# msg7086/x265-Yuuki-Asuna

Measured on AMD Instinct MI355X. Metric: encoded fps + bit-exact check, 4K preset=slow, 1/2/4/8 MI355X vs host AVX2, higher is better.
Workload: dtype u8; 1 GPU; 3840x2160 8-bit closed-loop frame pipeline (tier T2): lookahead -> exhaustive +-57 ME, 85 PUs/CTU -> subme 3 -> MC + DCT/quant/recon qp 27 -> deblock -> SAO (rdo) -> border -> next reference; parallelism=none (1 GPU), ctus_per_frame=2040

## Files before the change

x265-yuuki-asuna_amd/csrc/phase_kernels.hip:

```cpp
#include "common.h"
#include "tile_interp.h"

#include <cstdlib>

namespace x265hip {

struct PhaseArgs
{
    const uint8_t* src;
    uint8_t* dst;
    long strideB;
    int rows, tilesW, depth;
    size_t planeBytes;
};

__constant__ int8_t kPhaseChromaTaps[8][4] = {
    { 0, 64, 0, 0 }, { -2, 58, 10, -2 }, { -4, 54, 16, -2 }, { -6, 46, 28, -4 },
    { -4, 36, 36, -4 }, { -4, 28, 46, -6 }, { -2, 16, 54, -4 }, { -2, 10, 58, -2 } };

template <typename Px> __device__ __forceinline__ void phase_store(uint8_t* out, long strideB, const int (&d)[4][4])
{
#pragma unroll
    for (int y = 0; y < 4; y++)
    {
        uint32_t* o = reinterpret_cast<uint32_t*>(out + y * strideB);
        if (sizeof(Px) == 1)
            o[0] = (uint32_t)d[y][0] | ((uint32_t)d[y][1] << 8) | ((uint32_t)d[y][2] << 16) | ((uint32_t)d[y][3] << 24);
        else
        {
            o[0] = (uint32_t)d[y][0] | ((uint32_t)d[y][1] << 16);
            o[1] = (uint32_t)d[y][2] | ((uint32_t)d[y][3] << 16);
        }
    }
}

template <typename Px>
__global__ void __launch_bounds__(256) phase_luma_kernel(PhaseArgs a)
{
    constexpr int BPP = sizeof(Px);
    int bx, by;
    xcd_swizzle_2d(bx, by);
    const int tx = bx * 256 + threadIdx.x, ty = by + 1;
    if (tx >= a.tilesW) return;
    const long off = (long)(ty * 4) * a.strideB + (long)tx * 4 * BPP;
    const uint8_t* org = a.src + off;
    const int maxVal = (1 << a.depth) - 1, headRoom = 14 - a.depth;
    const int shiftPS = 6 - headRoom, offPS = -(8192 << shiftPS);
    const int shiftSP = 6 + headRoom, offSP = (1 << (shiftSP - 1)) + (8192 << 6);
    auto vtaps = [](const int yf, uint32_t (&cv)[4])
    {
        cv[0] = tile_sel3(yf, 0x0004ffffu, 0x0004ffffu, 0x00010000u); cv[1] = tile_sel3(yf, 0x003afff6u, 0x0028fff5u, 0x0011fffbu);
        cv[2] = tile_sel3(yf, 0xfffb0011u, 0xfff50028u, 0xfff6003au); cv[3] = tile_sel3(yf, 0x00000001u, 0xffff0004u, 0xffff0004u);
    };
#pragma unroll
    for (int xf = 0; xf < 4; xf++)
    {
        int col[11][4];
#pragma unroll
        for (int t = 0; t < 11; t++)
        {
            const uint8_t* rp = org + (long)(t - 3) * a.strideB;
            if (xf == 0)
            {
                if (BPP == 1) { const uint32_t w = ld_u32(rp); col[t][0] = w & 0xff; col[t][1] = (w >> 8) & 0xff; col[t][2] = (w >> 16) & 0xff; col[t][3] = w >> 24; }
                else { const uint32_t w0 = ld_u32(rp), w1 = ld_u32(rp + 4); col[t][0] = w0 & 0xffff; col[t][1] = w0 >> 16; col[t][2] = w1 & 0xffff; col[t][3] = w1 >> 16; }
            }
            else
                tile_hrow<BPP>(rp - 3 * BPP, xf, col[t]);
        }
        int d[4][4];
        if (xf)
        {
#pragma unroll
            for (int y = 0; y < 4; y++)
#pragma unroll
                for (int x = 0; x < 4; x++) d[y][x] = tile_clip16((col[y + 3][x] + 32) >> 6, maxVal);
            phase_store<Px>(a.dst + (size_t)(xf - 1) * a.planeBytes + off, a.strideB, d);
        }
        uint32_t pairs[10][4];
#pragma unroll
        for (int t = 0; t < 10; t++)
#pragma unroll
            for (int x = 0; x < 4; x++)
            {
                const uint32_t lo = xf ? (uint32_t)((col[t][x] + offPS) >> shiftPS) : (uint32_t)col[t][x];
                const uint32_t hi = xf ? (uint32_t)((col[t + 1][x] + offPS) >> shiftPS) : (uint32_t)col[t + 1][x];
                pairs[t][x] = __builtin_amdgcn_perm(hi, lo, 0x05040100u);
            }
#pragma unroll
        for (int yf = 1; yf < 4; yf++)
        {
            uint32_t cv[4];
            vtaps(yf, cv);
#pragma unroll
            for (int y = 0; y < 4; y++)
#pragma unroll
                for (int x = 0; x < 4; x++)
                {
                    int sum = 0;
#pragma unroll
                    for (int j = 0; j < 4; j++) sum = tile_dot2(pairs[y + 2 * j][x], cv[j], sum);
                    d[y][x] = xf ? tile_clip16((sum + offSP) >> shiftSP, maxVal) : tile_clip16((sum + 32) >> 6, maxVal);
                }
            phase_store<Px>(a.dst + (size_t)(yf * 4 + xf - 1) * a.planeBytes + off, a.strideB, d);
        }
    }
}

__device__ __forceinline__ uint32_t quad_xor1(uint32_t v) { return (uint32_t)dpp<0xB1>((int)v); }
__device__ __forceinline__ uint32_t quad_xor2(uint32_t v) { return (uint32_t)dpp<0x4E>((int)v); }

__device__ __forceinline__ void quad_transpose4(uint32_t (&p)[4], int l)
{
    const bool o1 = l & 1, o2 = l & 2;
    {
        const uint32_t a = quad_xor1(o1 ? p[0] : p[1]), b = quad_xor1(o1 ? p[2] : p[3]);
        if (o1) { p[0] = a; p[2] = b; } else { p[1] = a; p[3] = b; }
    }
    {
        const uint32_t a = quad_xor2(o2 ? p[0] : p[2]), b = quad_xor2(o2 ? p[1] : p[3]);
        if (o2) { p[0] = a; p[1] = b; } else { p[2] = a; p[3] = b; }
    }
}

template <typename Px> __device__ __forceinline__ void phase_store_wide(uint8_t* plane, long strideB, int ty, int tx, int lane, const int (&d)[4][4])
{
    if (sizeof(Px) == 1)
    {
        uint32_t p[4];
#pragma unroll
        for (int y = 0; y < 4; y++) p[y] = (uint32_t)d[y][0] | ((uint32_t)d[y][1] << 8) | ((uint32_t)d[y][2] << 16) | ((uint32_t)d[y][3] << 24);
        quad_transpose4(p, lane);
        uint4* o = reinterpret_cast<uint4*>(plane + (long)(ty * 4 + (lane & 3)) * strideB + (long)(tx & ~3) * 4);
        *o = make_uint4(p[0], p[1], p[2], p[3]);
    }
    else
    {
        uint32_t lo[4], hi[4];
#pragma unroll
        for (int y = 0; y < 4; y++) { lo[y] = (uint32_t)d[y][0] | ((uint32_t)d[y][1] << 16); hi[y] = (uint32_t)d[y][2] | ((uint32_t)d[y][3] << 16); }
        const bool odd = lane & 1;
#pragma unroll
        for (int r = 0; r < 4; r += 2)
        {
            const uint32_t sl = quad_xor1(odd ? lo[r] : lo[r + 1]), sh = quad_xor1(odd ? hi[r] : hi[r + 1]);
            const uint4 v = odd ? make_uint4(sl, sh, lo[r + 1], hi[r + 1]) : make_uint4(lo[r], hi[r], sl, sh);
            uint4* o = reinterpret_cast<uint4*>(plane + (long)(ty * 4 + r + (odd ? 1 : 0)) * strideB + (long)(tx & ~1) * 8);
            *o = v;
        }
    }
}

template <int BPP> __device__ __forceinline__ void tile_hrow_regs(const uint32_t* w, int xf, int (&out)[4])
{
    if (BPP == 1)
    {
        const uint32_t c03 = tile_sel3(xf, 0x3af604ffu, 0x28f504ffu, 0x11fb0100u), c47 = tile_sel3(xf, 0x0001fb11u, 0xff04f528u, 0xff04f63au);
        const uint32_t w0 = w[0] ^ 0x80808080u, w1 = w[1] ^ 0x80808080u, w2 = w[2] ^ 0x80808080u;
#pragma unroll
        for (int x = 0; x < 4; x++)
        {
            const uint32_t lo = x ? __builtin_amdgcn_alignbyte(w1, w0, x) : w0, hi = x ? __builtin_amdgcn_alignbyte(w2, w1, x) : w1;
            out[x] = __builtin_amdgcn_sdot4((int)hi, (int)c47, __builtin_amdgcn_sdot4((int)lo, (int)c03, 8192, false), false);
        }
    }
    else
    {
        const uint32_t cp[4] = { tile_sel3(xf, 0x0004ffffu, 0x0004ffffu, 0x00010000u), tile_sel3(xf, 0x003afff6u, 0x0028fff5u, 0x0011fffbu),
                                 tile_sel3(xf, 0xfffb0011u, 0xfff50028u, 0xfff6003au), tile_sel3(xf, 0x00000001u, 0xffff0004u, 0xffff0004u) };
#pragma unroll
        for (int x = 0; x < 4; x++)
        {
            int sacc = 0;
#pragma unroll
            for (int j = 0; j < 4; j++)
            {
                const int k = (x >> 1) + j;
                sacc = tile_dot2((x & 1) ? __builtin_amdgcn_alignbyte(w[k + 1], w[k], 2) : w[k], cp[j], sacc);
            }
            out[x] = sacc;
        }
    }
}

template <typename Px, bool XF0>
__device__ __forceinline__ void phase_column_set(const PhaseArgs& a, const uint32_t (&raw)[11][sizeof(Px) == 1 ? 3 : 6], int xf, int ty, int tx, int lane, bool live)
{
    constexpr int BPP = sizeof(Px);
    const int maxVal = (1 << a.depth) - 1, headRoom = 14 - a.depth;
    const int shiftPS = 6 - headRoom, offPS = -(8192 << shiftPS);
    const int shiftSP = 6 + headRoom, offSP = (1 << (shiftSP - 1)) + (8192 << 6);
    int d[4][4];
    uint32_t pairs[10][4], prev[4] = { 0, 0, 0, 0 };
#pragma unroll
    for (int t = 0; t < 11; t++)
    {
        int col[4];
        if (XF0)
        {
            if (BPP == 1)
            {
                const uint32_t w = __builtin_amdgcn_alignbyte(raw[t][1], raw[t][0], 3);
                col[0] = w & 0xff; col[1] = (w >> 8) & 0xff; col[2] = (w >> 16) & 0xff; col[3] = w >> 24;
            }
            else
            {
                col[0] = raw[t][1] >> 16; col[1] = raw[t][2] & 0xffff; col[2] = raw[t][2] >> 16; col[3] = raw[t][3] & 0xffff;
            }
        }
        else
        {
            tile_hrow_regs<BPP>(raw[t], xf, col);
            if (t >= 3 && t < 7)
#pragma unroll
                for (int x = 0; x < 4; x++) d[t - 3][x] = tile_clip16((col[x] + 32) >> 6, maxVal);
        }
#pragma unroll
        for (int x = 0; x < 4; x++)
        {
            const uint32_t cur = XF0 ? (uint32_t)col[x] : (uint32_t)((col[x] + offPS) >> shiftPS);
            if (t) pairs[t - 1][x] = __builtin_amdgcn_perm(cur, prev[x], 0x05040100u);
            prev[x] = cur;
        }
    }
    if (!XF0 && live) phase_store_wide<Px>(a.dst + (size_t)(xf - 1) * a.planeBytes, a.strideB, ty, tx, lane, d);
#pragma unroll 1
    for (int yf = 1; yf < 4; yf++)
    {
        const uint32_t cv[4] = { tile_sel3(yf, 0x0004ffffu, 0x0004ffffu, 0x00010000u), tile_sel3(yf, 0x003afff6u, 0x0028fff5u, 0x0011fffbu),
                                 tile_sel3(yf, 0xfffb0011u, 0xfff50028u, 0xfff6003au), tile_sel3(yf, 0x00000001u, 0xffff0004u, 0xffff0004u) };
#pragma unroll
        for (int y = 0; y < 4; y++)
#pragma unroll
            for (int x = 0; x < 4; x++)
            {
                int sum = 0;
#pragma unroll
                for (int j = 0; j < 4; j++) sum = tile_dot2(pairs[y + 2 * j][x], cv[j], sum);
                d[y][x] = XF0 ? tile_clip16((sum + 32) >> 6, maxVal) : tile_clip16((sum + offSP) >> shiftSP, maxVal);
            }
        if (live) phase_store_wide<Px>(a.dst + (size_t)(yf * 4 + xf - 1) * a.planeBytes, a.strideB, ty, tx, lane, d);
    }
}

template <typename Px>
__device__ __forceinline__ void phase_luma_wide_body(const PhaseArgs& a)
{
    constexpr int BPP = sizeof(Px), NW = BPP == 1 ? 3 : 6;
    const int lane = threadIdx.x & 63;
    int bx, by;
    xcd_swizzle_2d(bx, by);
    const int tx = bx * 256 + threadIdx.x, ty = by + 1;
    const bool live = tx < a.tilesW;
    const int txl = live ? tx : a.tilesW - 4 + (tx & 3);
    const uint8_t* org = a.src + (long)(ty * 4) * a.strideB + (long)txl * 4 * BPP;
    uint32_t raw[11][NW];
#pragma unroll
    for (int t = 0; t < 11; t++)
#pragma unroll
        for (int k = 0; k < NW; k++) raw[t][k] = ld_u32(org + (long)(t - 3) * a.strideB - 3 * BPP + 4 * k);
    phase_column_set<Px, true>(a, raw, 0, ty, tx, lane, live);
#pragma unroll 1
    for (int xf = 1; xf < 4; xf++)
        phase_column_set<Px, false>(a, raw, xf, ty, tx, lane, live);
}
template <typename Px> __global__ void __launch_bounds__(256) phase_luma_wide_kernel(PhaseArgs a) { phase_luma_wide_body<Px>(a); }

template <typename Px>
__global__ void __launch_bounds__(256) phase_chroma_kernel(PhaseArgs a)
{
    constexpr int BPP = sizeof(Px);
    int bx, by;
    xcd_swizzle_2d(bx, by);
    const int tx = bx * 256 + threadIdx.x, ty = by + 1;
    if (tx >= a.tilesW) return;
    const long off = (long)(ty * 4) * a.strideB + (long)tx * 4 * BPP;
    const int maxVal = (1 << a.depth) - 1, headRoom = 14 - a.depth;
    const int shiftPS = 6 - headRoom, offPS = -(8192 << shiftPS);
    const int shiftSP = 6 + headRoom, offSP = (1 << (shiftSP - 1)) + (8192 << 6);
    int s[7][7];
#pragma unroll
    for (int r = 0; r < 7; r++)
    {
        const uint8_t* rp = a.src + off + (long)(r - 1) * a.strideB - BPP;
        if (BPP == 1)
        {
            const uint32_t w0 = ld_u32(rp), w1 = ld_u32(rp + 4);
            s[r][0] = w0 & 0xff; s[r][1] = (w0 >> 8) & 0xff; s[r][2] = (w0 >> 16) & 0xff; s[r][3] = w0 >> 24;
            s[r][4] = w1 & 0xff; s[r][5] = (w1 >> 8) & 0xff; s[r][6] = (w1 >> 16) & 0xff;
        }
        else
        {
            const uint32_t w0 = ld_u32(rp), w1 = ld_u32(rp + 4), w2 = ld_u32(rp + 8), w3 = ld_u32(rp + 12);
            s[r][0] = w0 & 0xffff; s[r][1] = w0 >> 16; s[r][2] = w1 & 0xffff; s[r][3] = w1 >> 16;
            s[r][4] = w2 & 0xffff; s[r][5] = w2 >> 16; s[r][6] = w3 & 0xffff;
        }
    }
#pragma unroll 1
    for (int xf = 0; xf < 8; xf++)
    {
        const int cx0 = kPhaseChromaTaps[xf][0], cx1 = kPhaseChromaTaps[xf][1], cx2 = kPhaseChromaTaps[xf][2], cx3 = kPhaseChromaTaps[xf][3];
        int col[7][4];
#pragma unroll
        for (int r = 0; r < 7; r++)
#pragma unroll
            for (int x = 0; x < 4; x++)
                col[r][x] = xf ? cx0 * s[r][x] + cx1 * s[r][x + 1] + cx2 * s[r][x + 2] + cx3 * s[r][x + 3] : s[r][x + 1];
        int d[4][4];
        if (xf)
        {
#pragma unroll
            for (int y = 0; y < 4; y++)
#pragma unroll
                for (int x = 0; x < 4; x++) d[y][x] = tile_clip16((col[y + 1][x] + 32) >> 6, maxVal);
            phase_store<Px>(a.dst + (size_t)(xf - 1) * a.planeBytes + off, a.strideB, d);
#pragma unroll
            for (int r = 0; r < 7; r++)
#pragma unroll
                for (int x = 0; x < 4; x++) col[r][x] = (int16_t)((col[r][x] + offPS) >> shiftPS);
        }
#pragma unroll 1
        for (int yf = 1; yf < 8; yf++)
        {
            const int cy0 = kPhaseChromaTaps[yf][0], cy1 = kPhaseChromaTaps[yf][1], cy2 = kPhaseChromaTaps[yf][2], cy3 = kPhaseChromaTaps[yf][3];
#pragma unroll
            for (int y = 0; y < 4; y++)
#pragma unroll
                for (int x = 0; x < 4; x++)
                {
                    const int sum = cy0 * col[y][x] + cy1 * col[y + 1][x] + cy2 * col[y + 2][x] + cy3 * col[y + 3][x];
                    d[y][x] = xf ? tile_clip16((sum + offSP) >> shiftSP, maxVal) : tile_clip16((sum + 32) >> 6, maxVal);
                }
            phase_store<Px>(a.dst + (size_t)(yf * 8 + xf - 1) * a.planeBytes + off, a.strideB, d);
        }
    }
}

}

using namespace x265hip;

int x265hip::phase_planes_launch(int depth, int chroma, const void* src, void* dst, intptr_t stride, int rows, size_t plane_bytes, hipStream_t s)
{
    const int bpp = depth == 8 ? 1 : 2;
    PhaseArgs a;
    a.src = (const uint8_t*)src; a.dst = (uint8_t*)dst; a.strideB = (long)stride * bpp; a.rows = rows;
    a.tilesW = (int)(stride / 4); a.depth = depth; a.planeBytes = plane_bytes;
    const dim3 gridL((a.tilesW + 255) / 256, rows / 4 - 3);
    if (chroma)
    {
        if (bpp == 1) hipLaunchKernelGGL(phase_chroma_kernel<uint8_t>, gridL, dim3(256), 0, s, a);
        else hipLaunchKernelGGL(phase_chroma_kernel<uint16_t>, gridL, dim3(256), 0, s, a);
    }
    else
    {
        static const int force = getenv("X265HIP_PHASE_KERNEL") ? atoi(getenv("X265HIP_PHASE_KERNEL")) : 0;
        const bool wideOk = !(a.tilesW & 3) && !(((uintptr_t)dst | plane_bytes) & 15);
        const bool wide = wideOk && (force == 2 || (force != 1 && bpp == 2));
        if (wide)
        {
            if (bpp == 1) hipLaunchKernelGGL(phase_luma_wide_kernel<uint8_t>, gridL, dim3(256), 0, s, a);
            else hipLaunchKernelGGL(phase_luma_wide_kernel<uint16_t>, gridL, dim3(256), 0, s, a);
        }
        else if (bpp == 1) hipLaunchKernelGGL(phase_luma_kernel<uint8_t>, gridL, dim3(256), 0, s, a);
        else hipLaunchKernelGGL(phase_luma_kernel<uint16_t>, gridL, dim3(256), 0, s, a);
    }
    return check_hip(hipGetLastError(), "phase_planes launch");
}

extern "C" int x265hip_phase_planes(const x265hip_phase_planes_params* p, void* stream)
{
    if (!p || !p->src || !p->dst) { set_error("phase_planes: NULL argument"); return X265HIP_EINVAL; }
    if (p->depth != 8 && p->depth != 10 && p->depth != 12) { set_error("phase_planes: depth %d", p->depth); return X265HIP_EINVAL; }
    const int bpp = p->depth == 8 ? 1 : 2;
    if (p->stride <= 0 || p->rows <= 0 || (p->rows & 3) || ((p->stride * bpp) & 3) || (p->stride & 3))
    { set_error("phase_planes: stride %ld / rows %d must be positive multiples of 4", (long)p->stride, p->rows); return X265HIP_EINVAL; }
    if ((uintptr_t)p->dst & 3) { set_error("phase_planes: dst must be 4-byte aligned"); return X265HIP_EINVAL; }
    if (p->rows / 4 > 65535 || p->rows < 16) { set_error("phase_planes: %d rows", p->rows); return X265HIP_EINVAL; }
    int rc = ensure_device();
    if (rc) return rc;
    return phase_planes_launch(p->depth, p->chroma, p->src, p->dst, p->stride, p->rows, (size_t)p->stride * p->rows * bpp, (hipStream_t)stream);
}
```

Measured before the change: 659.4 frames/s.

## Add dedicated 8-bit luma phase kernel using packed dot products

Adds a specialized 8-bit luma subpel phase-plane kernel that computes horizontal filters with sdot4 on byte-aligned words and vertical filters with sdot2 on packed 16-bit pairs. It uses packed arithmetic-shift-clip-to-u8 instructions to produce all 15 phase planes in one pass over an 11-row window. This is meant to replace the generic templated per-pixel arithmetic for the default 8-bit path and cut ALU and register cost. The risk is bit-exactness in the bias and offset handling, plus higher register pressure from the pairs array.

Measured after the change: 673.0 frames/s (median of 6 runs). 2.1% higher.

```diff
diff --git a/x265-yuuki-asuna_amd/csrc/phase_kernels.hip b/x265-yuuki-asuna_amd/csrc/phase_kernels.hip
--- a/x265-yuuki-asuna_amd/csrc/phase_kernels.hip
+++ b/x265-yuuki-asuna_amd/csrc/phase_kernels.hip
@@ -266,6 +266,85 @@
 }
 template <typename Px> __global__ void __launch_bounds__(256) phase_luma_wide_kernel(PhaseArgs a) { phase_luma_wide_body<Px>(a); }
 
+typedef unsigned short phase_v2u16 __attribute__((ext_vector_type(2)));
+template <int S> __device__ __forceinline__ uint32_t ashr_clip_pack4(const int (&d)[4])
+{
+    const phase_v2u16 v = { __builtin_amdgcn_ashr_pk_u8_i32(d[0], d[1], S), __builtin_amdgcn_ashr_pk_u8_i32(d[2], d[3], S) };
+    return __builtin_bit_cast(uint32_t, v);
+}
+
+__global__ void __launch_bounds__(256) phase_luma8_kernel(PhaseArgs a)
+{
+    int bx, by;
+    xcd_swizzle_2d(bx, by);
+    const int tx = bx * 256 + threadIdx.x, y0 = 4 + by * 4;
+    if (tx >= a.tilesW) return;
+    const uint32_t laneB = threadIdx.x * 4;
+    const uint8_t* __restrict__ org = a.src + (long)(y0 - 3) * a.strideB + (long)bx * 1024 - 3;
+    uint8_t* out = a.dst + (long)y0 * a.strideB + (long)bx * 1024;
+    uint32_t raw[11][3];
+#pragma unroll
+    for (int t = 0; t < 11; t++)
+#pragma unroll
+        for (int k = 0; k < 3; k++) raw[t][k] = ld_u32(org + (long)t * a.strideB + 4 * k + laneB);
+    uint32_t pairs[4][10][4];
+    uint32_t prev[4][4];
+#pragma unroll
+    for (int t = 0; t < 11; t++)
+    {
+        const uint32_t cen = __builtin_amdgcn_alignbyte(raw[t][1], raw[t][0], 3);
+        const uint32_t w0 = raw[t][0] ^ 0x80808080u, w1 = raw[t][1] ^ 0x80808080u, w2 = raw[t][2] ^ 0x80808080u;
+        uint32_t lo[4], hi[4];
+#pragma unroll
+        for (int x = 0; x < 4; x++)
+        {
+            lo[x] = x ? __builtin_amdgcn_alignbyte(w1, w0, x) : w0;
+            hi[x] = x ? __builtin_amdgcn_alignbyte(w2, w1, x) : w1;
+        }
+        if (t)
+#pragma unroll
+            for (int x = 0; x < 4; x++)
+                pairs[0][t - 1][x] = __builtin_amdgcn_perm(cen, prev[0][0], 0x0c000c00u | (uint32_t)x | ((uint32_t)(4 + x) << 16));
+        prev[0][0] = cen;
+#pragma unroll
+        for (int xf = 1; xf < 4; xf++)
+        {
+            const uint32_t c03 = tile_sel3(xf, 0x3af604ffu, 0x28f504ffu, 0x11fb0100u), c47 = tile_sel3(xf, 0x0001fb11u, 0xff04f528u, 0xff04f63au);
+            int hs[4];
+#pragma unroll
+            for (int x = 0; x < 4; x++)
+            {
+                hs[x] = __builtin_amdgcn_sdot4((int)hi[x], (int)c47, __builtin_amdgcn_sdot4((int)lo[x], (int)c03, 8192 + 32, true), false);
+                if (t) pairs[xf][t - 1][x] = __builtin_amdgcn_perm((uint32_t)hs[x], prev[xf][x], 0x05040100u);
+                prev[xf][x] = (uint32_t)hs[x];
+            }
+            if (t >= 3 && t < 7)
+                *reinterpret_cast<uint32_t*>(out + (size_t)(xf - 1) * a.planeBytes + (long)(t - 3) * a.strideB + laneB) = ashr_clip_pack4<6>(hs);
+        }
+        if (t < 7) continue;
+        uint8_t* line = out + (long)(t - 7) * a.strideB;
+#pragma unroll
+        for (int yf = 1; yf < 4; yf++)
+        {
+            const uint32_t cv[4] = { tile_sel3(yf, 0x0004ffffu, 0x0004ffffu, 0x00010000u), tile_sel3(yf, 0x003afff6u, 0x0028fff5u, 0x0011fffbu),
+                                     tile_sel3(yf, 0xfffb0011u, 0xfff50028u, 0xfff6003au), tile_sel3(yf, 0x00000001u, 0xffff0004u, 0xffff0004u) };
+#pragma unroll
+            for (int xf = 0; xf < 4; xf++)
+            {
+                int d[4];
+#pragma unroll
+                for (int x = 0; x < 4; x++)
+                {
+                    d[x] = __builtin_amdgcn_sdot2(__builtin_bit_cast(tile_v2i16, pairs[xf][t - 7][x]), __builtin_bit_cast(tile_v2i16, cv[0]), xf ? 0 : 32, true);
+#pragma unroll
+                    for (int j = 1; j < 4; j++) d[x] = tile_dot2(pairs[xf][t - 7 + 2 * j][x], cv[j], d[x]);
+                }
+                *reinterpret_cast<uint32_t*>(line + (size_t)(yf * 4 + xf - 1) * a.planeBytes + laneB) = xf ? ashr_clip_pack4<12>(d) : ashr_clip_pack4<6>(d);
+            }
+        }
+    }
+}
+
 template <typename Px>
 __global__ void __launch_bounds__(256) phase_chroma_kernel(PhaseArgs a)
 {
@@ -357,7 +436,8 @@
         static const int force = getenv("X265HIP_PHASE_KERNEL") ? atoi(getenv("X265HIP_PHASE_KERNEL")) : 0;
         const bool wideOk = !(a.tilesW & 3) && !(((uintptr_t)dst | plane_bytes) & 15);
         const bool wide = wideOk && (force == 2 || (force != 1 && bpp == 2));
-        if (wide)
+        if (bpp == 1 && force != 1 && force != 2) hipLaunchKernelGGL(phase_luma8_kernel, gridL, dim3(256), 0, s, a);
+        else if (wide)
         {
             if (bpp == 1) hipLaunchKernelGGL(phase_luma_wide_kernel<uint8_t>, gridL, dim3(256), 0, s, a);
             else hipLaunchKernelGGL(phase_luma_wide_kernel<uint16_t>, gridL, dim3(256), 0, s, a);
```
